# thiviyanT/torch-rgcn

Hardware: AMD Instinct MI355X
Metric: edges/s/GPU (fwd+bwd) 2-layer RGCN, 1M nodes/10M edges/50 rels, h=16 (higher is better)
Workload: dtype f32; 1 GPU; S1: N=1000000 nodes, E=10000000 base triples, R0=50 relations (layer R=101), M=21000000 messages/layer, hidden=16, 2 NC layers (horizontal, vertical), fwd+bwd, learnable X

## Files before the change

include/rgcn_hip.h:

```cpp
#ifndef RGCN_HIP_H
#define RGCN_HIP_H

#include <stdint.h>

#ifdef __cplusplus
extern "C" {
#endif

#define RGCN_API __attribute__((visibility("default")))

#define RGCN_OK 0
#define RGCN_EINVAL 1
#define RGCN_ENOMEM 2
#define RGCN_ERANGE 3
#define RGCN_EHIP 4
#define RGCN_EUNSUPPORTED 5

#define RGCN_CHUNK 16

RGCN_API const char *rgcn_version(void);
RGCN_API const char *rgcn_last_error(void);
RGCN_API const char *rgcn_csrc_sha(void);
RGCN_API int rgcn_poison_lds(void *stream);
RGCN_API int rgcn_set_option(const char *name, int32_t value);
// ... 77 lines not shown
                           int32_t d_out, int32_t flags, void *stream);

RGCN_API int rgcn_pack_w16_f32(const float *W, float *Wp, int32_t R, void *stream);
RGCN_API int rgcn_pack_w_blocks_f32(const float *W, float *Wp, int32_t R, int32_t d_in, int32_t d_out, void *stream);

RGCN_API int rgcn_spmm_scatter_f32(const float *X, const float *Wp, float *Y, const int32_t *p_src,
                                   const float *p_val, const int32_t *p_pos, const int32_t *chunk_rel,
                                   const int32_t *items, int64_t n_items, int32_t d, void *stream);
RGCN_API int rgcn_segment_sum_f32(const float *Y, const int32_t *rowptr, const float *bias, float *out,
                                  int64_t n_rows, int32_t d, int32_t flags, void *stream);
RGCN_API int rgcn_segment_gather_sum_f32(const float *Y, const int32_t *perm, const int32_t *rowptr, const float *bias,
                                         float *out, int64_t n_rows, int32_t d, int32_t flags, void *stream);
RGCN_API int rgcn_segment_gather_sum_units_f32(const float *Y, const int32_t *perm, const int32_t *units, int64_t n_units,
                                               int64_t n_split, const float *bias, float *out, int64_t n_rows, int32_t d,
                                               int32_t flags, void *stream);

RGCN_API int rgcn_wgrad_f32(const float *X, const float *G, float *dW, const int32_t *p_src,
                            const int32_t *p_dst, const float *p_val, const int32_t *chunk_rel,
                            const int32_t *items, int64_t n_items, int64_t n_dst, int64_t n_src, int32_t R,
                            int32_t d_in, int32_t d_out, void *stream);

RGCN_API int rgcn_wgrad_tiled_f32(const float *X, const float *G, float *dW, const int32_t *p_src,
                                  const int32_t *p_dst, const float *p_val, const int32_t *chunk_rel,
                                  const int32_t *run_ptr, int64_t n_tiles, int32_t tile_rows, int64_t n_dst,
                                  int64_t n_src, int32_t R, int32_t d_in, int32_t d_out,
                                  int32_t tiles_per_item, void *stream);

#define RGCN_F_DW_ATOMIC 4
#define RGCN_F_TRANSPOSE_W 8
#define RGCN_F_DIAG4 16
#define RGCN_F_PARTIAL 32
#define RGCN_F_ACCUMULATE 64
RGCN_API int64_t rgcn_bwd_fused_scratch_floats(int64_t n_tiles, int32_t R);
RGCN_API int64_t rgcn_bwd_lean_slot_bytes(int64_t n_chunks);
RGCN_API int rgcn_bwd_lean_prepare_f32(const int32_t *p_pack, const int32_t *chunk_rel, int64_t n_chunks, void *slots, int32_t *hdr,
                                       void *stream);
RGCN_API int rgcn_bwd_lean_prepare_unpacked_f32(const int32_t *p_src, const int32_t *p_dst, const float *p_val, int32_t tile_rows,
                                                const int32_t *chunk_rel, int64_t n_chunks, void *slots, int32_t *hdr, void *stream);
RGCN_API int rgcn_bwd_lean_supported(int32_t tile_rows);
RGCN_API int rgcn_bwd_lean_f32(const float *G, const float *X, const float *Wt_packed, float *dX, float *dW, float *scratch,
                               const void *slots, const int32_t *hdr, const int32_t *run_ptr, int64_t n_tiles, int32_t tile_rows,
                               int64_t n_dst, int32_t R, int32_t flags, void *stream);
RGCN_API int32_t rgcn_bwd_blk_max_rows(int32_t R, int32_t flags);
RGCN_API int rgcn_bwd_blk_supported(int32_t tile_rows, int32_t R, int32_t flags);
RGCN_API int64_t rgcn_bwd_blk_rec_bytes(int64_t n_chunks);
RGCN_API int rgcn_bwd_blk_prepare_f32(const int32_t *p_pack, const int32_t *p_src, const int32_t *p_dst, const float *p_val,
                                      int32_t tile_rows, const int32_t *chunk_rel, int64_t n_chunks, void *rec, void *stream);
RGCN_API int rgcn_bwd_blk_f32(const float *G, const float *X, const float *Wt_packed, float *dX, float *dW, const void *rec,
                              const int32_t *run_ptr, int64_t n_tiles, int32_t tile_rows, int64_t n_dst, int32_t R, int32_t flags,
                              float *dbias, int64_t n_src, const int32_t *units, int64_t n_units, int64_t n_split, void *stream);
RGCN_API int32_t rgcn_bwd_own_waves(void);
RGCN_API int32_t rgcn_bwd_own_units(void);
RGCN_API int32_t rgcn_bwd_own_max_rows(void);
RGCN_API int rgcn_bwd_own_f32(const float *G, const float *X, const float *Wt_packed, float *dX, float *dW, const void *rec,
                              const int32_t *own_ptr, const int32_t *unit_rel, int64_t n_tiles, int32_t tile_rows, int64_t n_dst,
                              int32_t R, int32_t flags, float *dbias, int64_t n_src, void *stream);
RGCN_API int rgcn_bwd_own_bf16(const uint16_t *G, const uint16_t *X, const float *Wt_packed, uint16_t *dX, float *dW, const void *rec,
                               const int32_t *own_ptr, const int32_t *unit_rel, int64_t n_tiles, int32_t tile_rows, int64_t n_dst,
                               int32_t R, int32_t flags, float *dbias, int64_t n_src, void *stream);
RGCN_API int64_t rgcn_softwin_tmp_bytes(int64_t n);
RGCN_API int rgcn_softwin_order(const int32_t *dst, const int32_t *src, const int32_t *rel, const uint8_t *alive, int64_t M, int64_t n_dst,
                                int64_t n_src, int32_t R, int32_t tile_rows, uint64_t *keys, uint64_t *keys_sorted, int32_t *order,
                                int32_t *order_sorted, int32_t *bucket_cnt, int32_t *bucket_base, int32_t *bucket_first, void *tmp,
                                int64_t tmp_bytes, void *stream);
RGCN_API int rgcn_softwin_fill(const int32_t *dst, const int32_t *src, const float *val, const uint64_t *keys_sorted, const int32_t *order_sorted,
                               int64_t n_live, int64_t n_dst, int64_t n_src, int32_t R, int32_t tile_rows, const int32_t *bucket_base,
                               const int32_t *bucket_first, int64_t m_pad, const int32_t *parts, const int32_t *unit_base,
                               const int32_t *unit_owner, const int32_t *unit_local, int32_t own_waves, int32_t *s_src, int32_t *s_dst, float *s_val,
                               uint64_t *ckeys, uint64_t *ckeys_sorted, int32_t *cidx, int32_t *cidx_sorted, int32_t *crel, int32_t *group_cnt,
                               int32_t *p_src, int32_t *p_dst, float *p_val, int32_t *chunk_rel, int32_t *group_ptr, void *tmp, int64_t tmp_bytes,
                               void *stream);
RGCN_API int32_t rgcn_spmm_blk_max_rows(void);
RGCN_API int rgcn_spmm_blk_f32(const float *X, const float *W_packed, const float *bias, float *out, const void *rec,
                               const int32_t *run_ptr, int64_t n_tiles, int32_t tile_rows, int64_t n_dst, int32_t R, int32_t flags,
                               const int32_t *units, int64_t n_units, int64_t n_split, void *stream);
RGCN_API int rgcn_spmm_blk_bf16(const uint16_t *X, const float *W_packed, const float *bias, uint16_t *out, float *scratch, const void *rec,
                                const int32_t *run_ptr, int64_t n_tiles, int32_t tile_rows, int64_t n_dst, int64_t n_src, int32_t R,
                                int32_t flags, const int32_t *units, int64_t n_units, int64_t n_split, void *stream);
RGCN_API int rgcn_spmm_bf16(const uint16_t *X, const float *W_packed, const float *bias, uint16_t *out, float *scratch,
                            const int32_t *p_pack, const int32_t *chunk_rel, const int32_t *units, int64_t n_units, int64_t n_split,
                            int32_t tile_rows, int64_t n_dst, int64_t n_src, int32_t d_in, int32_t d_out, int32_t flags, void *stream);
RGCN_API int rgcn_wgrad_bf16(const uint16_t *X, const uint16_t *G, float *dW, const int32_t *p_src, const int32_t *p_dst,
                             const float *p_val, const int32_t *chunk_rel, const int32_t *items, int64_t n_items, int32_t R,
                             int32_t d_in, int32_t d_out, void *stream);
RGCN_API int rgcn_colsum_bf16(const uint16_t *G, float *db, float *scratch, int64_t n, int32_t d, void *stream);
RGCN_API int rgcn_block_spmm_bf16(const uint16_t *X, const float *blocks, const float *bias, uint16_t *out, float *scratch,
                                  const int32_t *units, const int32_t *rowptr, int64_t n_units, int64_t n_split, const int32_t *e_src,
                                  const int32_t *e_rel, const float *e_val, int64_t n_rows, int32_t n_rel_blocks, int32_t nb, int32_t bi,
                                  int32_t bo, int32_t flags, void *stream);
RGCN_API int rgcn_block_wgrad_bf16(const uint16_t *X, const uint16_t *G, float *dblocks, const int32_t *p_src, const int32_t *p_dst,
                                   const float *p_val, const int32_t *chunk_rel, const int32_t *items, int64_t n_items,
                                   int32_t n_rel_blocks, int32_t nb, int32_t bi, int32_t bo, void *stream);
RGCN_API int rgcn_diag_spmm_bf16(const uint16_t *X, const float *w, const float *bias, uint16_t *out, float *scratch,
                                 const int32_t *rowptr_units, int64_t n_units, int64_t n_split, const int32_t *e_src, const int32_t *e_rel,
                                 const float *e_val, int64_t n_rows, int32_t R, int32_t d, void *stream);
RGCN_API int rgcn_diag_wgrad_bf16(const uint16_t *X, const uint16_t *G, float *dw, const int32_t *p_src, const int32_t *p_dst,
                                  const float *p_val, const int32_t *chunk_rel, const int32_t *items, int64_t n_items, int32_t R, int32_t d,
                                  void *stream);
RGCN_API int rgcn_bwd_scatter_dw_f32(const float *G, const float *X, const float *Wt_packed, float *Y, float *dW,
                                     const int32_t *p_src, const int32_t *p_dst, const float *p_val,
                                     const int32_t *chunk_rel, const int32_t *items, int64_t n_items, int32_t R, int32_t d,
                                     int32_t flags, void *stream);
RGCN_API int rgcn_pack_w16t_f32(const float *W, float *Wp, int32_t R, void *stream);
RGCN_API int rgcn_pack_w16_pair_f32(const float *W, float *Wp, float *Wtp, int32_t R, void *stream);

RGCN_API int rgcn_featureless_fwd_f32(const float *table, const float *bias, float *out, const int32_t *p_src,
                                      const int32_t *p_dst, const float *p_val, const int32_t *chunk_rel,
                                      const int32_t *units, int64_t n_units, int64_t n_split, int32_t tile_rows,
                                      int64_t n_dst, int64_t n_src, int32_t R, int32_t d_out, void *stream);

RGCN_API int rgcn_spmm_csr_d16_supported(int32_t R);
RGCN_API int rgcn_spmm_csr_d16_f32(const float *X, const float *W, const float *bias, float *out, const int32_t *units, int64_t n_units,
// ... 152 lines not shown
```

torch-rgcn_amd/csrc/rgcn_bwd_own.hip:

```cpp
#include <stdlib.h>
#include <string.h>

#include <algorithm>

#include "rgcn_device.h"

namespace {

constexpr int OWN_REC = 176;
constexpr int OWN_REC_ROWS = 128;
constexpr int OWN_REC_HDR = 160;
constexpr int OWN_LDS_MAX = 160 * 1024;
#ifndef RGCN_OWN_NW
#define RGCN_OWN_NW 16
#define RGCN_OWN_K 8
#define RGCN_OWN_U 2
#endif
constexpr int OWN_NW = RGCN_OWN_NW;
constexpr int OWN_K = RGCN_OWN_K;
constexpr int OWN_U = RGCN_OWN_U;
constexpr int OWN_MAX_ROWS = (OWN_LDS_MAX - OWN_NW * BW_SCR2 * 4 - 64) / 192;

typedef float own_acc32 __attribute__((ext_vector_type(32)));

size_t bwd_own_lds(int rows) { return (size_t)rows * 192 + (size_t)OWN_NW * BW_SCR2 * 4 + 64; }

template <bool RELU, int NW, int K, int ABL = 0, bool BF = false>
__global__ __launch_bounds__(64 * NW) void bwd_own_d16_kernel(
    const float *__restrict__ G, const float *__restrict__ X, const float *__restrict__ Wtp, float *__restrict__ dX,
    float *__restrict__ dWout, const char *__restrict__ rec, const int *__restrict__ own_ptr, int n_tiles, int tile_rows, int n_dst,
    float *__restrict__ dbias, int n_src, const int *__restrict__ unit_rel) {
  constexpr int U = OWN_U, NT = 64 * NW;
  constexpr int TQ = (OWN_MAX_ROWS * 4 + NT - 1) / NT;
  static_assert(K <= 9, "8 indexed accumulators + 1");
  constexpr bool EXT = K == 9;
  extern __shared__ __attribute__((aligned(16))) char lds[];
  const int tid = threadIdx.x;
  const int wave = __builtin_amdgcn_readfirstlane(tid >> 6), lane = tid & 63;
  const unsigned xt_off = (unsigned)tile_rows * 128u;
  const unsigned xs_off = (unsigned)tile_rows * 192u;
  float4 *dxz = reinterpret_cast<float4 *>(lds);
  const double2 *dxd2 = reinterpret_cast<const double2 *>(lds);
  float4 *xt4 = reinterpret_cast<float4 *>(lds + xt_off);
  float *xs = reinterpret_cast<float *>(lds + xs_off) + wave * BW_SCR2;

  int t = blockIdx.x;
  int row0 = t * tile_rows;
  int nrows = min(tile_rows, n_dst - row0);
  int c0 = own_ptr[(size_t)t * NW + wave], c1 = own_ptr[(size_t)t * NW + wave + 1];
  c0 = __builtin_amdgcn_readfirstlane(c0);
  c1 = __builtin_amdgcn_readfirstlane(c1);
  float4 gs = make_float4(0.f, 0.f, 0.f, 0.f);
  const long long g_n4 = dbias ? (long long)n_src * 4 : 0, g_step = (long long)gridDim.x * NT;
  long long g_i = (long long)blockIdx.x * NT + tid;
#pragma unroll
  for (int q = 0; q < TQ; ++q) {
    const int idx = tid + q * NT;
    if (idx < tile_rows * 4) {
      float4 x0 = make_float4(0.f, 0.f, 0.f, 0.f);
      if (idx < nrows * 4) {
        if constexpr (BF) x0 = bf16x4_widen(reinterpret_cast<const uint2 *>(X)[(size_t)row0 * 4 + idx]);
        else x0 = reinterpret_cast<const float4 *>(X + (size_t)row0 * 16)[idx];
      }
      xt4[idx] = x0;
    }
  }
  for (int i = tid; i < tile_rows * 8; i += NT) dxz[i] = make_float4(0.f, 0.f, 0.f, 0.f);
  __syncthreads();

  const int m = lane & 15, k = lane >> 4;
  const unsigned kofs = (unsigned)k << 4;
  const unsigned dx_lane = (unsigned)m * 8u;
  const unsigned xrd = xt_off + (unsigned)m * 4u;
  float *xs_wr = xs + m * 16 + 4 * ((k + (m >> 2)) & 3);
  const float *xs_rd = xs + (4 * k) * 16 + 4 * (((m >> 2) + k) & 3) + (m & 3);
  const unsigned slot_lane = (unsigned)m * 8u;
  const unsigned rows_lane = (unsigned)OWN_REC_ROWS + (unsigned)k * 8u;
  const unsigned w_lane = (unsigned)lane * 16u;

  own_acc32 accs;
#pragma unroll
  for (int i = 0; i < 32; ++i) accs[i] = 0.f;
  f32x4 acc8 = f32x4{0.f, 0.f, 0.f, 0.f};

  uint2 sl_n[U], rw_n[U];
  int hd_n[U];
  auto request_idx = [&](int c, int last) {
#pragma unroll
    for (int j = 0; j < U; ++j) {
      const int cc = min(c + j, last);
      const char *r = rec + (size_t)cc * OWN_REC;
      sl_n[j] = *reinterpret_cast<const uint2 *>(r + slot_lane);
      rw_n[j] = *reinterpret_cast<const uint2 *>(r + rows_lane);
      hd_n[j] = *reinterpret_cast<const int *>(r + OWN_REC_HDR);
    }
  };
  if (c0 < c1) request_idx(c0, c1 - 1);

  for (;;) {
    const int last = c1 - 1;
    for (int c = c0; c < c1; c += U) {
      unsigned w0_[U];
      uint2 rw_[U];
      float v_[U];
      int hd_[U];
      float4 g_[U], w_[U];
#pragma unroll
// ... 60 lines not shown
#pragma unroll
          for (int t4 = 0; t4 < 4; ++t4) bv[jj][t4] = xs_rd[16 * t4];
#pragma unroll
          for (int t4 = 0; t4 < 4; ++t4) av[jj][t4] = *reinterpret_cast<const float *>(lds + (xrd + ro[j][t4]));
          asm volatile("" ::: "memory");
        }
#pragma unroll
        for (int jj = 0; jj < P; ++jj) {
          if (h + jj >= U) break;
          const int lr = (ABL & 4) ? 0 : (int)((unsigned)hd_[h + jj] >> 16);
          const bool ext = EXT && lr >= 8;
          const int li = 4 * (lr & 7);
          const f32x4 in0 = f32x4{accs[li], accs[li + 1], accs[li + 2], accs[li + 3]};
          f32x4 aw = EXT ? f32x4{ext ? acc8[0] : in0[0], ext ? acc8[1] : in0[1], ext ? acc8[2] : in0[2], ext ? acc8[3] : in0[3]} : in0;
#pragma unroll
          for (int t4 = 0; t4 < 4; ++t4) aw = __builtin_amdgcn_mfma_f32_16x16x4f32(av[jj][t4], bv[jj][t4], aw, 0, 0, 0);
          accs[li] = ext ? in0[0] : aw[0];
          accs[li + 1] = ext ? in0[1] : aw[1];
          accs[li + 2] = ext ? in0[2] : aw[2];
          accs[li + 3] = ext ? in0[3] : aw[3];
          if (EXT) acc8 = f32x4{ext ? aw[0] : acc8[0], ext ? aw[1] : acc8[1], ext ? aw[2] : acc8[2], ext ? aw[3] : acc8[3]};
        }
      }
#pragma unroll
      for (int j = 0; j < U && !(ABL & 8); ++j)
#pragma unroll
        for (int e = 0; e < 4; ++e)
          __hip_atomic_fetch_add(static_cast<double *>(__builtin_assume_aligned(lds + (dx_lane + 2u * ro[j][e]), 8)), (double)acc[j][e], __ATOMIC_RELAXED,
                                 __HIP_MEMORY_SCOPE_WORKGROUP);
      __builtin_amdgcn_sched_barrier(0);
    }
    const int tn = t + (int)gridDim.x;
    int c0n = 0, c1n = 0, row0n = 0, nrn = 0;
    float4 xn[TQ];
#pragma unroll
    for (int q = 0; q < TQ; ++q) xn[q] = make_float4(0.f, 0.f, 0.f, 0.f);
    if (tn < n_tiles) {
      row0n = tn * tile_rows;
      nrn = min(tile_rows, n_dst - row0n);
      c0n = __builtin_amdgcn_readfirstlane(own_ptr[(size_t)tn * NW + wave]);
      c1n = __builtin_amdgcn_readfirstlane(own_ptr[(size_t)tn * NW + wave + 1]);
#pragma unroll
      for (int q = 0; q < TQ; ++q)
        if (tid + q * NT < nrn * 4) {
          if constexpr (BF) {
            const uint2 u = reinterpret_cast<const uint2 *>(X)[(size_t)row0n * 4 + tid + q * NT];
            xn[q] = make_float4(__uint_as_float(u.x), __uint_as_float(u.y), 0.f, 0.f);
          } else {
            xn[q] = reinterpret_cast<const float4 *>(X + (size_t)row0n * 16)[tid + q * NT];
          }
        }
      if (c0n < c1n) request_idx(c0n, c1n - 1);
    }
    float4 gn = make_float4(0.f, 0.f, 0.f, 0.f);
    if (g_i < g_n4) {
      if constexpr (BF) gn = bf16x4_widen(reinterpret_cast<const uint2 *>(G)[g_i]);
      else gn = reinterpret_cast<const float4 *>(G)[g_i];
    }
    g_i += g_step;
    lds_barrier();
    gs.x += gn.x; gs.y += gn.y; gs.z += gn.z; gs.w += gn.w;
#pragma unroll
    for (int q = 0; q < TQ; ++q) asm volatile("" : "+v"(xn[q].x), "+v"(xn[q].y), "+v"(xn[q].z), "+v"(xn[q].w));
#pragma unroll
    for (int q = 0; q < TQ; ++q) {
      const int idx = tid + q * NT;
      if (idx < nrows * 4) {
        const double2 d0 = dxd2[2 * idx], d1 = dxd2[2 * idx + 1];
        float4 a = make_float4((float)d0.x, (float)d0.y, (float)d1.x, (float)d1.y);
        if (RELU) {
          const float4 x = xt4[idx];
          a.x = x.x > 0.f ? a.x : 0.f; a.y = x.y > 0.f ? a.y : 0.f; a.z = x.z > 0.f ? a.z : 0.f; a.w = x.w > 0.f ? a.w : 0.f;
        }
        if constexpr (BF) reinterpret_cast<uint2 *>(dX)[(size_t)row0 * 4 + idx] = bf16x4_round(a);
        else reinterpret_cast<float4 *>(dX + (size_t)row0 * 16)[idx] = a;
      }
    }
    if (tn >= n_tiles) break;
#pragma unroll
    for (int q = 0; q < TQ; ++q) {
      const int idx = tid + q * NT;
      if (idx < tile_rows * 4) {
        dxz[2 * idx] = make_float4(0.f, 0.f, 0.f, 0.f);
        dxz[2 * idx + 1] = make_float4(0.f, 0.f, 0.f, 0.f);
        if constexpr (BF) xt4[idx] = bf16x4_widen(uint2{__float_as_uint(xn[q].x), __float_as_uint(xn[q].y)});
        else xt4[idx] = xn[q];
      }
    }
    lds_barrier();
    t = tn; row0 = row0n; nrows = nrn; c0 = c0n; c1 = c1n;
  }
  if (dbias) {
    for (; g_i < g_n4; g_i += g_step) {
      float4 gn;
      if constexpr (BF) gn = bf16x4_widen(reinterpret_cast<const uint2 *>(G)[g_i]);
      else gn = reinterpret_cast<const float4 *>(G)[g_i];
      gs.x += gn.x; gs.y += gn.y; gs.z += gn.z; gs.w += gn.w;
    }
#pragma unroll
    for (int sft = 4; sft < 64; sft <<= 1) {
      gs.x += __shfl_xor(gs.x, sft); gs.y += __shfl_xor(gs.y, sft); gs.z += __shfl_xor(gs.z, sft); gs.w += __shfl_xor(gs.w, sft);
    }
    __syncthreads();
    if (lane < 4) *reinterpret_cast<float4 *>(xs + 4 * lane) = gs;
    __syncthreads();
    if (tid < 16) {
      float a = 0.f;
      const float *all = reinterpret_cast<const float *>(lds + xs_off);
      for (int i = 0; i < NW; ++i) a += all[i * BW_SCR2 + tid];
      atomicAdd(dbias + tid, a);
    }
  }
#pragma unroll
  for (int li = 0; li < K; ++li) {
    const int r = __builtin_amdgcn_readfirstlane(unit_rel[wave * K + li]);
    if (r >= 0) {
      float *o = dWout + (size_t)r * 256 + (4 * k) * 16 + m;
      atomicAdd(o, li < 8 ? accs[(4 * li) & 31] : acc8[0]);
      atomicAdd(o + 16, li < 8 ? accs[(4 * li + 1) & 31] : acc8[1]);
      atomicAdd(o + 32, li < 8 ? accs[(4 * li + 2) & 31] : acc8[2]);
      atomicAdd(o + 48, li < 8 ? accs[(4 * li + 3) & 31] : acc8[3]);
    }
  }
}

}

extern "C" int32_t rgcn_bwd_own_waves(void) { return OWN_NW; }
extern "C" int32_t rgcn_bwd_own_units(void) { return OWN_NW * OWN_K; }
extern "C" int32_t rgcn_bwd_own_max_rows(void) { return OWN_MAX_ROWS; }

extern "C" int rgcn_bwd_own_f32(const float *G, const float *X, const float *Wt_packed, float *dX, float *dW, const void *rec,
                                const int32_t *own_ptr, const int32_t *unit_rel, int64_t n_tiles, int32_t tile_rows, int64_t n_dst,
                                int32_t R, int32_t flags, float *dbias, int64_t n_src, void *stream) {
  if (!G || !X || !Wt_packed || !dX || !dW || !rec || !own_ptr || !unit_rel || n_tiles <= 0 || tile_rows <= 0 || n_dst <= 0 || R <= 0 ||
      R > 0xFFFF || n_dst > INT32_MAX || n_tiles * (int64_t)OWN_NW >= INT32_MAX) {
    rgcn_set_error("bwd_own: bad argument");
    return RGCN_EINVAL;
  }
  if (tile_rows > rgcn_bwd_own_max_rows()) {
    rgcn_set_error("bwd_own: tiles of at most %d rows (got %d)", rgcn_bwd_own_max_rows(), tile_rows);
    return RGCN_EUNSUPPORTED;
  }
  if (dbias && (n_src <= 0 || n_src >= (int64_t(1) << 29))) { rgcn_set_error("bwd_own: dbias needs 0 < n_src < 2^29"); return RGCN_EINVAL; }
  hipStream_t st = (hipStream_t)stream;
  int dev = 0, n_cu = 0;
  HIP_TRY(launch_device(&dev, &n_cu));
  HIP_TRY(zero_dw_dbias_async(dW, (size_t)R, dbias, st));
  const size_t lds = bwd_own_lds(tile_rows);
  const unsigned n_blocks = (unsigned)std::min<int64_t>(n_tiles, n_cu);
  auto launch = [&](auto k) -> hipError_t {
    constexpr auto kern = decltype(k)::value;
    hipError_t e = allow_lds<kern>(dev, lds, OWN_LDS_MAX);
    if (e != hipSuccess) return e;
    hipLaunchKernelGGL(kern, dim3(n_blocks), dim3(64 * OWN_NW), lds, st, G, X, Wt_packed, dX, dW, static_cast<const char *>(rec), own_ptr, (int)n_tiles,
                       tile_rows, (int)n_dst, dbias, (int)n_src, unit_rel);
    return hipGetLastError();
  };
#ifdef RGCN_ABLATIONS
  {
    const int ABLV = rgcn_option_value(RGCN_OPT_BWD_ABL);
    if (ABLV == 2) HIP_TRY(launch(kern_c<bwd_own_d16_kernel<false, OWN_NW, OWN_K, 2>>));
    else if (ABLV == 4) HIP_TRY(launch(kern_c<bwd_own_d16_kernel<false, OWN_NW, OWN_K, 4>>));
    else if (ABLV == 8) HIP_TRY(launch(kern_c<bwd_own_d16_kernel<false, OWN_NW, OWN_K, 8>>));
    else if (ABLV == 16) HIP_TRY(launch(kern_c<bwd_own_d16_kernel<false, OWN_NW, OWN_K, 16>>));
    else if (ABLV == 6) HIP_TRY(launch(kern_c<bwd_own_d16_kernel<false, OWN_NW, OWN_K, 6>>));
    else HIP_TRY(launch(kern_c<bwd_own_d16_kernel<false, OWN_NW, OWN_K, 0>>));
    return RGCN_OK;
  }
#endif
  if (flags & RGCN_F_RELU) HIP_TRY(launch(kern_c<bwd_own_d16_kernel<true, OWN_NW, OWN_K>>));
  else HIP_TRY(launch(kern_c<bwd_own_d16_kernel<false, OWN_NW, OWN_K>>));
  return RGCN_OK;
}

extern "C" int rgcn_bwd_own_bf16(const uint16_t *G, const uint16_t *X, const float *Wt_packed, uint16_t *dX, float *dW, const void *rec,
                                 const int32_t *own_ptr, const int32_t *unit_rel, int64_t n_tiles, int32_t tile_rows, int64_t n_dst,
                                 int32_t R, int32_t flags, float *dbias, int64_t n_src, void *stream) {
  if (!G || !X || !Wt_packed || !dX || !dW || !rec || !own_ptr || !unit_rel || n_tiles <= 0 || tile_rows <= 0 || n_dst <= 0 || R <= 0 ||
      R > 0xFFFF || n_dst > INT32_MAX || n_tiles * (int64_t)OWN_NW >= INT32_MAX || n_src <= 0 || n_src >= (int64_t(1) << 26) || flags != 0) {
    rgcn_set_error("bwd_own_bf16: bad argument (the records address G rows as src << 6 in 32 bits: n_src < 2^26; no flags)");
    return RGCN_EINVAL;
  }
  if (tile_rows > rgcn_bwd_own_max_rows()) {
    rgcn_set_error("bwd_own_bf16: tiles of at most %d rows (got %d)", rgcn_bwd_own_max_rows(), tile_rows);
    return RGCN_EUNSUPPORTED;
  }
  hipStream_t st = (hipStream_t)stream;
  int dev = 0, n_cu = 0;
  HIP_TRY(launch_device(&dev, &n_cu));
  HIP_TRY(zero_dw_dbias_async(dW, (size_t)R, dbias, st));
  const size_t lds = bwd_own_lds(tile_rows);
  const unsigned n_blocks = (unsigned)std::min<int64_t>(n_tiles, n_cu);
  auto launch = [&](auto k) -> hipError_t {
    constexpr auto kern = decltype(k)::value;
    hipError_t e = allow_lds<kern>(dev, lds, OWN_LDS_MAX);
    if (e != hipSuccess) return e;
    hipLaunchKernelGGL(kern, dim3(n_blocks), dim3(64 * OWN_NW), lds, st, reinterpret_cast<const float *>(G), reinterpret_cast<const float *>(X),
                       Wt_packed, reinterpret_cast<float *>(dX), dW, static_cast<const char *>(rec), own_ptr, (int)n_tiles, tile_rows, (int)n_dst,
                       dbias, (int)n_src, unit_rel);
    return hipGetLastError();
  };
  HIP_TRY(launch(kern_c<bwd_own_d16_kernel<false, OWN_NW, OWN_K, 0, true>>));
  return RGCN_OK;
}
```

torch-rgcn_amd/torch_rgcn/_native.py:

```python
import ctypes
import re
import threading
import os

import numpy as np
import torch

from . import routes

_LIB_PATH = os.environ.get("RGCN_HIP_LIB") or os.path.join(os.path.dirname(os.path.abspath(__file__)), "lib", "librgcn_hip.so")
_HEADER_PATH = os.path.join(os.path.dirname(os.path.abspath(__file__)), "..", "..", "include", "rgcn_hip.h")
_lib = None

OK, EINVAL, ENOMEM, ERANGE, EHIP, EUNSUPPORTED = range(6)
CHUNK = 16

c_i64 = ctypes.c_int64
_CTYPES = {"int": ctypes.c_int, "int32_t": ctypes.c_int32, "int64_t": ctypes.c_int64, "uint64_t": ctypes.c_uint64}


class NativeLibraryError(RuntimeError):
    pass


# ... 1332 lines not shown
            if cached[2] == 0:
                cached = (None, plan.n_tiles, 0)
        plan._blk_units = cached
    return cached


def _lean_plan(plan):
    lean = getattr(plan, "_lean", None)
    if lean is None:
        n_chunks = plan.chunk_rel.shape[0]
        dev = plan.chunk_rel.device
        slots = torch.empty(int(lib().rgcn_bwd_lean_slot_bytes(n_chunks)) + 16, device=dev, dtype=torch.uint8)
        hdr = torch.empty(max(n_chunks, 1), device=dev, dtype=torch.int32)
        with _on(dev):
            if plan.pack is not None:
                _check(lib().rgcn_bwd_lean_prepare_f32(_dp(plan.pack), _dp(plan.chunk_rel), n_chunks, _dp(slots), _dp(hdr), _stream(dev)),
                       "bwd_lean_prepare")
            else:
                _check(lib().rgcn_bwd_lean_prepare_unpacked_f32(_dp(plan.src), _dp(plan.dst), _dp(plan.val), plan.tile_rows,
                                                                _dp(plan.chunk_rel), n_chunks, _dp(slots), _dp(hdr), _stream(dev)),
                       "bwd_lean_prepare_unpacked")
        lean = plan._lean = (slots, hdr)
    return lean


def _blk_rec(plan):
    rec = getattr(plan, "_blk_rec", None)
    if rec is None:
        n_chunks = plan.chunk_rel.shape[0]
        dev = plan.chunk_rel.device
        rec = torch.empty(int(lib().rgcn_bwd_blk_rec_bytes(n_chunks)) + 16, device=dev, dtype=torch.uint8)
        packed = plan.pack is not None and plan.tile_rows <= 255
        with _on(dev):
            _check(lib().rgcn_bwd_blk_prepare_f32(_dp(plan.pack) if packed else None, _dp(plan.src), _dp(plan.dst), _dp(plan.val),
                                                  plan.tile_rows, _dp(plan.chunk_rel), n_chunks, _dp(rec), _stream(dev)),
                   "bwd_blk_prepare")
        plan._blk_rec = rec
    return rec


def bwd_own_geometry():
    L = lib()
    nw = int(L.rgcn_bwd_own_waves())
    return nw, int(L.rgcn_bwd_own_units()) // nw, int(L.rgcn_bwd_own_max_rows())


def bwd_own_rows(n_nodes, device=None):
    if n_nodes < _BLK_MIN_NODES:
        return 0
    cap = min(bwd_own_geometry()[2], int(routes.get("own_rows_cap", "767")))
    return _even_tile_rows(n_nodes, cap, device)


def bwd_own(G, X, W, plan, relu=False, want_db=False):
    _req(G, "grad_output"); _req(X, "features"); _req(W, "weights")
    assert W.shape[1:] == (16, 16) and G.shape == (plan.n_src, 16) and X.shape == (plan.n_dst, 16) and W.shape[0] == plan.num_rels
    assert getattr(plan, "own_ptr", None) is not None, "bwd_own: a plan made with build_softwin_plan(own_waves=...)"
    dev = G.device
    Wtp = pack_w16t(W)
    dX = torch.empty((plan.n_dst, 16), device=dev, dtype=torch.float32)
    buf = torch.empty(W.numel() + 16, device=dev, dtype=torch.float32)
    dW, db = buf[:W.numel()].view_as(W), buf[W.numel():]
    rec = _blk_rec(plan)
    with _on(dev), _timed("bwd_fused"):
        _check(lib().rgcn_bwd_own_f32(_dp(G), _dp(X), _dp(Wtp), _dp(dX), _dp(dW), _dp(rec), _dp(plan.own_ptr), _dp(plan.unit_rel),
                                      plan.n_tiles, plan.tile_rows, plan.n_dst, W.shape[0], F_RELU if relu else 0,
                                      _dp(db) if want_db else None, plan.n_src, _stream(dev)), "bwd_own")
    return (dX, dW, db if want_db else None)


def bwd_own_bf16(G, X, W, plan, relu=False, want_db=False):
    _req(G, "grad_output", torch.bfloat16); _req(X, "features", torch.bfloat16); _req(W, "weights")
    assert W.shape[1:] == (16, 16) and G.shape == (plan.n_src, 16) and X.shape == (plan.n_dst, 16) and W.shape[0] == plan.num_rels
    assert getattr(plan, "own_ptr", None) is not None, "bwd_own_bf16: a plan made with build_softwin_plan(own_waves=...)"
    dev = G.device
    Wtp = pack_w16t(W)
    dX = torch.empty((plan.n_dst, 16), device=dev, dtype=torch.bfloat16)
    buf = torch.empty(W.numel() + 16, device=dev, dtype=torch.float32)
    dW, db = buf[:W.numel()].view_as(W), buf[W.numel():]
    rec = _blk_rec(plan)
    with _on(dev), _timed("bwd_own_bf16"):
        _check(lib().rgcn_bwd_own_bf16(_dp(G), _dp(X), _dp(Wtp), _dp(dX), _dp(dW), _dp(rec), _dp(plan.own_ptr), _dp(plan.unit_rel), plan.n_tiles,
                                       plan.tile_rows, plan.n_dst, W.shape[0], F_RELU if relu else 0, _dp(db) if want_db else None, plan.n_src,
                                       _stream(dev)), "bwd_own_bf16")
    return (dX, dW, db if want_db else None)


def bwd_fused_relu_ok(plan, diag4=False):
    return bool(_bwd_blk_plan(plan, diag4)) or bwd_fused_ok(plan, diag4)


def bwd_fused(G, X, W, plan, atomic=False, relu=False, want_db=False, diag4=False):
    _req(G, "grad_output"); _req(X, "features"); _req(W, "weights")
    assert W.shape[1:] == (16, 16) and G.shape == (plan.n_src, 16) and X.shape == (plan.n_dst, 16)
    dev = G.device
    Wtp = pack_w16t(W)
    dX = torch.empty((plan.n_dst, 16), device=dev, dtype=torch.float32)
    blk = _bwd_blk_plan(plan, diag4)
    if diag4 and not blk:
        raise NativeLibraryError("bwd_fused: diag4 needs the block-tile kernel (plan of tall tiles, non-deterministic mode)")
    db = None
    if blk and want_db:
        buf = torch.empty(W.numel() + 16, device=dev, dtype=torch.float32)
        dW, db = buf[:W.numel()].view_as(W), buf[W.numel():]
    else:
        dW = torch.empty_like(W)
    ret = (lambda: (dX, dW, db)) if want_db else (lambda: (dX, dW))
    scratch = None
    if not atomic:
        n = int(lib().rgcn_bwd_fused_scratch_floats(plan.n_tiles, W.shape[0]))
        scratch = torch.empty(n, device=dev, dtype=torch.float32)
    if blk:
        if not atomic:
            raise NativeLibraryError("bwd_fused: the block-tile plan (tall tiles) has no bit-reproducible kernel")
        rec = _blk_rec(plan)
        units, n_units, n_split = _blk_units(plan)
        with _on(dev), _timed("bwd_fused"):
            _check(lib().rgcn_bwd_blk_f32(_dp(G), _dp(X), _dp(Wtp), _dp(dX), _dp(dW), _dp(rec), _dp(plan.run_ptr), plan.n_tiles,
                                          plan.tile_rows, plan.n_dst, W.shape[0],
                                          (F_RELU if relu else 0) | (F_DIAG4 if diag4 else 0), _dp(db), plan.n_src, _dp(units),
                                          n_units, n_split, _stream(dev)), "bwd_blk")
        return ret()
    if not (lib().rgcn_bwd_lean_supported(plan.tile_rows) and W.shape[0] < 65536):
        raise NativeLibraryError(f"bwd_fused: no fused kernel for wave-owned tiles of {plan.tile_rows} rows (bwd_fused_ok)")
    slots, hdr = _lean_plan(plan)
    with _on(dev), _timed("bwd_fused"):
        _check(lib().rgcn_bwd_lean_f32(_dp(G), _dp(X), _dp(Wtp), _dp(dX), _dp(dW), _dp(scratch), _dp(slots), _dp(hdr),
                                       _dp(plan.run_ptr), plan.n_tiles, plan.tile_rows, plan.n_dst, W.shape[0],
                                       (F_DW_ATOMIC if atomic else 0) | (1 if relu else 0), _stream(dev)), "bwd_lean")
    return ret()


def bwd_fused_slabs_ok(plan):
    return bool(_bwd_blk_plan(plan)) and _blk_units(plan)[2] == 0 and getattr(plan, "tile_ptr", None) is not None


def bwd_fused_slabs(G, X, W, plan, n_slabs, after_slab):
# ... 495 lines not shown
```

Before: 6.636 billion edges/s.

## Replace dW/dbias atomics in owner backward with per-block partials plus reduce kernel

The owner-partitioned backward kernel now writes each block's per-unit dW accumulators and dbias partial sums to a scratch buffer instead of issuing global atomicAdds, and a new reduction kernel sums them per relation. This also drops the memset that zeroed dW/dbias up front. The dbias G streaming is split across up to TQ loads per tile iteration so the bias sum covers G in fewer passes. The cost is an extra kernel launch, a scratch allocation per call, and a reduce that scans all units for every relation.

```diff
diff --git a/include/rgcn_hip.h b/include/rgcn_hip.h
--- a/include/rgcn_hip.h
+++ b/include/rgcn_hip.h
@@ -153,12 +153,21 @@
 RGCN_API int32_t rgcn_bwd_own_waves(void);
 RGCN_API int32_t rgcn_bwd_own_units(void);
 RGCN_API int32_t rgcn_bwd_own_max_rows(void);
+RGCN_API int64_t rgcn_bwd_own_scratch_floats(int64_t n_tiles);
 RGCN_API int rgcn_bwd_own_f32(const float *G, const float *X, const float *Wt_packed, float *dX, float *dW, const void *rec,
                               const int32_t *own_ptr, const int32_t *unit_rel, int64_t n_tiles, int32_t tile_rows, int64_t n_dst,
                               int32_t R, int32_t flags, float *dbias, int64_t n_src, void *stream);
+RGCN_API int rgcn_bwd_own_part_f32(const float *G, const float *X, const float *Wt_packed, float *dX, float *dW, const void *rec,
+                                   const int32_t *own_ptr, const int32_t *unit_rel, int64_t n_tiles, int32_t tile_rows, int64_t n_dst,
+                                   int32_t R, int32_t flags, float *dbias, int64_t n_src, float *scratch, int64_t scratch_floats,
+                                   void *stream);
 RGCN_API int rgcn_bwd_own_bf16(const uint16_t *G, const uint16_t *X, const float *Wt_packed, uint16_t *dX, float *dW, const void *rec,
                                const int32_t *own_ptr, const int32_t *unit_rel, int64_t n_tiles, int32_t tile_rows, int64_t n_dst,
                                int32_t R, int32_t flags, float *dbias, int64_t n_src, void *stream);
+RGCN_API int rgcn_bwd_own_part_bf16(const uint16_t *G, const uint16_t *X, const float *Wt_packed, uint16_t *dX, float *dW, const void *rec,
+                                    const int32_t *own_ptr, const int32_t *unit_rel, int64_t n_tiles, int32_t tile_rows, int64_t n_dst,
+                                    int32_t R, int32_t flags, float *dbias, int64_t n_src, float *scratch, int64_t scratch_floats,
+                                    void *stream);
 RGCN_API int64_t rgcn_softwin_tmp_bytes(int64_t n);
 RGCN_API int rgcn_softwin_order(const int32_t *dst, const int32_t *src, const int32_t *rel, const uint8_t *alive, int64_t M, int64_t n_dst,
                                 int64_t n_src, int32_t R, int32_t tile_rows, uint64_t *keys, uint64_t *keys_sorted, int32_t *order,
diff --git a/torch-rgcn_amd/csrc/rgcn_bwd_own.hip b/torch-rgcn_amd/csrc/rgcn_bwd_own.hip
--- a/torch-rgcn_amd/csrc/rgcn_bwd_own.hip
+++ b/torch-rgcn_amd/csrc/rgcn_bwd_own.hip
@@ -2,6 +2,7 @@
 #include <string.h>
 
 #include <algorithm>
+#include <type_traits>
 
 #include "rgcn_device.h"
 
@@ -20,17 +21,24 @@
 constexpr int OWN_K = RGCN_OWN_K;
 constexpr int OWN_U = RGCN_OWN_U;
 constexpr int OWN_MAX_ROWS = (OWN_LDS_MAX - OWN_NW * BW_SCR2 * 4 - 64) / 192;
+constexpr int OWN_TQ = (OWN_MAX_ROWS * 4 + 64 * OWN_NW - 1) / (64 * OWN_NW);
+constexpr int OWN_UNITS = OWN_NW * OWN_K;
+constexpr int OWN_PART_BLOCK = OWN_UNITS * 256;
+#ifndef RGCN_OWN_AB
+#define RGCN_OWN_AB 0
+#endif
 
 typedef float own_acc32 __attribute__((ext_vector_type(32)));
 
 size_t bwd_own_lds(int rows) { return (size_t)rows * 192 + (size_t)OWN_NW * BW_SCR2 * 4 + 64; }
 
-template <bool RELU, int NW, int K, int ABL = 0, bool BF = false>
+template <bool RELU, int NW, int K, int ABL = 0, bool BF = false, bool PART = false>
 __global__ __launch_bounds__(64 * NW) void bwd_own_d16_kernel(
     const float *__restrict__ G, const float *__restrict__ X, const float *__restrict__ Wtp, float *__restrict__ dX,
     float *__restrict__ dWout, const char *__restrict__ rec, const int *__restrict__ own_ptr, int n_tiles, int tile_rows, int n_dst,
-    float *__restrict__ dbias, int n_src, const int *__restrict__ unit_rel) {
+    float *__restrict__ dbias, int n_src, const int *__restrict__ unit_rel, float *__restrict__ part, int g_share) {
   constexpr int U = OWN_U, NT = 64 * NW;
+  typedef std::conditional_t<BF, uint2, float4> g_raw;
   constexpr int TQ = (OWN_MAX_ROWS * 4 + NT - 1) / NT;
   static_assert(K <= 9, "8 indexed accumulators + 1");
   constexpr bool EXT = K == 9;
@@ -53,6 +61,13 @@
   float4 gs = make_float4(0.f, 0.f, 0.f, 0.f);
   const long long g_n4 = dbias ? (long long)n_src * 4 : 0, g_step = (long long)gridDim.x * NT;
   long long g_i = (long long)blockIdx.x * NT + tid;
+  const g_raw *Gq = reinterpret_cast<const g_raw *>(G);
+  auto gs_add = [&](const g_raw &v) {
+    float4 f;
+    if constexpr (BF) f = bf16x4_widen(v);
+    else f = v;
+    gs.x += f.x; gs.y += f.y; gs.z += f.z; gs.w += f.w;
+  };
 #pragma unroll
   for (int q = 0; q < TQ; ++q) {
     const int idx = tid + q * NT;
@@ -219,14 +234,18 @@
         }
       if (c0n < c1n) request_idx(c0n, c1n - 1);
     }
-    float4 gn = make_float4(0.f, 0.f, 0.f, 0.f);
-    if (g_i < g_n4) {
-      if constexpr (BF) gn = bf16x4_widen(reinterpret_cast<const uint2 *>(G)[g_i]);
-      else gn = reinterpret_cast<const float4 *>(G)[g_i];
-    }
-    g_i += g_step;
+    g_raw gn[TQ];
+#pragma unroll
+    for (int q = 0; q < TQ; ++q) {
+      gn[q] = g_raw{};
+      if (q < g_share) {
+        if (g_i < g_n4) gn[q] = Gq[g_i];
+        g_i += g_step;
+      }
+    }
     lds_barrier();
-    gs.x += gn.x; gs.y += gn.y; gs.z += gn.z; gs.w += gn.w;
+#pragma unroll
+    for (int q = 0; q < TQ; ++q) gs_add(gn[q]);
 #pragma unroll
     for (int q = 0; q < TQ; ++q) asm volatile("" : "+v"(xn[q].x), "+v"(xn[q].y), "+v"(xn[q].z), "+v"(xn[q].w));
 #pragma unroll
@@ -258,12 +277,7 @@
     t = tn; row0 = row0n; nrows = nrn; c0 = c0n; c1 = c1n;
   }
   if (dbias) {
-    for (; g_i < g_n4; g_i += g_step) {
-      float4 gn;
-      if constexpr (BF) gn = bf16x4_widen(reinterpret_cast<const uint2 *>(G)[g_i]);
-      else gn = reinterpret_cast<const float4 *>(G)[g_i];
-      gs.x += gn.x; gs.y += gn.y; gs.z += gn.z; gs.w += gn.w;
-    }
+    for (; g_i < g_n4; g_i += g_step) gs_add(Gq[g_i]);
 #pragma unroll
     for (int sft = 4; sft < 64; sft <<= 1) {
       gs.x += __shfl_xor(gs.x, sft); gs.y += __shfl_xor(gs.y, sft); gs.z += __shfl_xor(gs.z, sft); gs.w += __shfl_xor(gs.w, sft);
@@ -275,13 +289,19 @@
       float a = 0.f;
       const float *all = reinterpret_cast<const float *>(lds + xs_off);
       for (int i = 0; i < NW; ++i) a += all[i * BW_SCR2 + tid];
-      atomicAdd(dbias + tid, a);
+      if constexpr (PART) part[(size_t)gridDim.x * (NW * K * 256) + (size_t)blockIdx.x * 16 + tid] = a;
+      else atomicAdd(dbias + tid, a);
     }
   }
 #pragma unroll
   for (int li = 0; li < K; ++li) {
     const int r = __builtin_amdgcn_readfirstlane(unit_rel[wave * K + li]);
-    if (r >= 0) {
+    if constexpr (PART) {
+      if (r >= 0) {
+        float *o = part + ((size_t)blockIdx.x * (NW * K) + wave * K + li) * 256 + lane * 4;
+        *reinterpret_cast<f32x4 *>(o) = li < 8 ? f32x4{accs[(4 * li) & 31], accs[(4 * li + 1) & 31], accs[(4 * li + 2) & 31], accs[(4 * li + 3) & 31]} : acc8;
+      }
+    } else if (r >= 0) {
       float *o = dWout + (size_t)r * 256 + (4 * k) * 16 + m;
       atomicAdd(o, li < 8 ? accs[(4 * li) & 31] : acc8[0]);
       atomicAdd(o + 16, li < 8 ? accs[(4 * li + 1) & 31] : acc8[1]);
@@ -291,83 +311,160 @@
   }
 }
 
-}
-
-extern "C" int32_t rgcn_bwd_own_waves(void) { return OWN_NW; }
-extern "C" int32_t rgcn_bwd_own_units(void) { return OWN_NW * OWN_K; }
-extern "C" int32_t rgcn_bwd_own_max_rows(void) { return OWN_MAX_ROWS; }
-
-extern "C" int rgcn_bwd_own_f32(const float *G, const float *X, const float *Wt_packed, float *dX, float *dW, const void *rec,
-                                const int32_t *own_ptr, const int32_t *unit_rel, int64_t n_tiles, int32_t tile_rows, int64_t n_dst,
-                                int32_t R, int32_t flags, float *dbias, int64_t n_src, void *stream) {
+__global__ __launch_bounds__(256) void own_reduce_kernel(const float *__restrict__ part, const int *__restrict__ unit_rel, float *__restrict__ dW,
+                                                         float *__restrict__ dbias, int n_blocks, int n_units, int R) {
+  __shared__ float4 red[16 * 16];
+  float *redf = reinterpret_cast<float *>(red);
+  const int r = blockIdx.x, q = blockIdx.y, tid = threadIdx.x;
+  const int col = tid & 15, s = tid >> 4;
+  if (r == R) {
+    if (q) return;
+    const float *gsp = part + (size_t)n_blocks * n_units * 256;
+    float a = 0.f;
+    for (int b = s; b < n_blocks; b += 16) a += gsp[(size_t)b * 16 + col];
+    redf[s * 16 + col] = a;
+    __syncthreads();
+    if (tid < 16) {
+      float t = 0.f;
+      for (int i = 0; i < 16; ++i) t += redf[i * 16 + tid];
+      dbias[tid] = t;
+    }
+    return;
+  }
+  const float4 *p = reinterpret_cast<const float4 *>(part) + 16 * q + col;
+  const size_t bstep = (size_t)n_units * 64;
+  float4 a = make_float4(0.f, 0.f, 0.f, 0.f);
+  for (int u = 0; u < n_units; ++u) {
+    if (unit_rel[u] != r) continue;
+    const float4 *pu = p + (size_t)u * 64;
+    int b = s;
+    for (; b + 48 < n_blocks; b += 64) {
+      const float4 v0 = pu[(size_t)b * bstep], v1 = pu[(size_t)(b + 16) * bstep], v2 = pu[(size_t)(b + 32) * bstep], v3 = pu[(size_t)(b + 48) * bstep];
+      a.x += v0.x; a.y += v0.y; a.z += v0.z; a.w += v0.w;
+      a.x += v1.x; a.y += v1.y; a.z += v1.z; a.w += v1.w;
+      a.x += v2.x; a.y += v2.y; a.z += v2.z; a.w += v2.w;
+      a.x += v3.x; a.y += v3.y; a.z += v3.z; a.w += v3.w;
+    }
+    for (; b < n_blocks; b += 16) {
+      const float4 v = pu[(size_t)b * bstep];
+      a.x += v.x; a.y += v.y; a.z += v.z; a.w += v.w;
+    }
+  }
+  red[s * 16 + col] = a;
+  __syncthreads();
+  if (tid < 64) {
+    const int e = tid >> 4;
+    float t = 0.f;
+    for (int i = 0; i < 16; ++i) t += redf[(i * 16 + col) * 4 + e];
+    dW[(size_t)r * 256 + (4 * q + e) * 16 + col] = t;
+  }
+}
+
+int64_t own_scratch_floats(int64_t n_tiles, int n_cu) { return std::min<int64_t>(n_tiles, n_cu) * (OWN_PART_BLOCK + 16); }
+
+template <bool BF>
+int bwd_own_run(const char *who, const void *G, const void *X, const float *Wt_packed, void *dX, float *dW, const void *rec, const int32_t *own_ptr,
+                const int32_t *unit_rel, int64_t n_tiles, int32_t tile_rows, int64_t n_dst, int32_t R, int32_t flags, float *dbias, int64_t n_src,
+                float *scratch, int64_t scratch_floats, void *stream) {
   if (!G || !X || !Wt_packed || !dX || !dW || !rec || !own_ptr || !unit_rel || n_tiles <= 0 || tile_rows <= 0 || n_dst <= 0 || R <= 0 ||
-      R > 0xFFFF || n_dst > INT32_MAX || n_tiles * (int64_t)OWN_NW >= INT32_MAX) {
-    rgcn_set_error("bwd_own: bad argument");
+      R > 0xFFFF || n_dst > INT32_MAX || n_tiles * (int64_t)OWN_NW >= INT32_MAX || ((BF || dbias) && n_src <= 0) || n_src >= (int64_t(1) << 26) ||
+      (BF && flags != 0)) {
+    rgcn_set_error("%s: bad argument (the records address G rows as src << 6 in 32 bits: n_src < 2^26%s)", who, BF ? "; no flags" : "");
     return RGCN_EINVAL;
   }
   if (tile_rows > rgcn_bwd_own_max_rows()) {
-    rgcn_set_error("bwd_own: tiles of at most %d rows (got %d)", rgcn_bwd_own_max_rows(), tile_rows);
+    rgcn_set_error("%s: tiles of at most %d rows (got %d)", who, rgcn_bwd_own_max_rows(), tile_rows);
     return RGCN_EUNSUPPORTED;
   }
-  if (dbias && (n_src <= 0 || n_src >= (int64_t(1) << 29))) { rgcn_set_error("bwd_own: dbias needs 0 < n_src < 2^29"); return RGCN_EINVAL; }
   hipStream_t st = (hipStream_t)stream;
   int dev = 0, n_cu = 0;
   HIP_TRY(launch_device(&dev, &n_cu));
-  HIP_TRY(zero_dw_dbias_async(dW, (size_t)R, dbias, st));
+  if (scratch && scratch_floats < own_scratch_floats(n_tiles, n_cu)) {
+    rgcn_set_error("%s: scratch of %lld floats, rgcn_bwd_own_scratch_floats(%lld) = %lld", who, (long long)scratch_floats, (long long)n_tiles,
+                   (long long)own_scratch_floats(n_tiles, n_cu));
+    return RGCN_EINVAL;
+  }
+  if (RGCN_OWN_AB & 1) scratch = nullptr;
+#ifdef RGCN_ABLATIONS
+  const int ABLV = BF ? 0 : rgcn_option_value(RGCN_OPT_BWD_ABL);
+  if (ABLV) scratch = nullptr;
+#endif
+  if (!scratch) HIP_TRY(zero_dw_dbias_async(dW, (size_t)R, dbias, st));
   const size_t lds = bwd_own_lds(tile_rows);
   const unsigned n_blocks = (unsigned)std::min<int64_t>(n_tiles, n_cu);
+  const int64_t g_cover = ((n_tiles + n_blocks - 1) / n_blocks) * (int64_t)n_blocks * 64 * OWN_NW;
+  const int g_share = (RGCN_OWN_AB & 2) || !dbias ? 1 : (int)std::min<int64_t>(OWN_TQ, std::max<int64_t>(1, (n_src * 4 + g_cover - 1) / g_cover));
   auto launch = [&](auto k) -> hipError_t {
     constexpr auto kern = decltype(k)::value;
     hipError_t e = allow_lds<kern>(dev, lds, OWN_LDS_MAX);
     if (e != hipSuccess) return e;
-    hipLaunchKernelGGL(kern, dim3(n_blocks), dim3(64 * OWN_NW), lds, st, G, X, Wt_packed, dX, dW, static_cast<const char *>(rec), own_ptr, (int)n_tiles,
-                       tile_rows, (int)n_dst, dbias, (int)n_src, unit_rel);
+    hipLaunchKernelGGL(kern, dim3(n_blocks), dim3(64 * OWN_NW), lds, st, static_cast<const float *>(G), static_cast<const float *>(X), Wt_packed,
+                       static_cast<float *>(dX), dW, static_cast<const char *>(rec), own_ptr, (int)n_tiles, tile_rows, (int)n_dst, dbias, (int)n_src,
+                       unit_rel, scratch, g_share);
     return hipGetLastError();
   };
+  if constexpr (BF) {
+    if (scratch) HIP_TRY(launch(kern_c<bwd_own_d16_kernel<false, OWN_NW, OWN_K, 0, true, true>>));
+    else HIP_TRY(launch(kern_c<bwd_own_d16_kernel<false, OWN_NW, OWN_K, 0, true>>));
+  } else {
 #ifdef RGCN_ABLATIONS
-  {
-    const int ABLV = rgcn_option_value(RGCN_OPT_BWD_ABL);
-    if (ABLV == 2) HIP_TRY(launch(kern_c<bwd_own_d16_kernel<false, OWN_NW, OWN_K, 2>>));
-    else if (ABLV == 4) HIP_TRY(launch(kern_c<bwd_own_d16_kernel<false, OWN_NW, OWN_K, 4>>));
-    else if (ABLV == 8) HIP_TRY(launch(kern_c<bwd_own_d16_kernel<false, OWN_NW, OWN_K, 8>>));
-    else if (ABLV == 16) HIP_TRY(launch(kern_c<bwd_own_d16_kernel<false, OWN_NW, OWN_K, 16>>));
-    else if (ABLV == 6) HIP_TRY(launch(kern_c<bwd_own_d16_kernel<false, OWN_NW, OWN_K, 6>>));
-    else HIP_TRY(launch(kern_c<bwd_own_d16_kernel<false, OWN_NW, OWN_K, 0>>));
-    return RGCN_OK;
-  }
+    if (ABLV) {
+      if (ABLV == 2) HIP_TRY(launch(kern_c<bwd_own_d16_kernel<false, OWN_NW, OWN_K, 2>>));
+      else if (ABLV == 4) HIP_TRY(launch(kern_c<bwd_own_d16_kernel<false, OWN_NW, OWN_K, 4>>));
+      else if (ABLV == 8) HIP_TRY(launch(kern_c<bwd_own_d16_kernel<false, OWN_NW, OWN_K, 8>>));
+      else if (ABLV == 16) HIP_TRY(launch(kern_c<bwd_own_d16_kernel<false, OWN_NW, OWN_K, 16>>));
+      else if (ABLV == 6) HIP_TRY(launch(kern_c<bwd_own_d16_kernel<false, OWN_NW, OWN_K, 6>>));
+      else HIP_TRY(launch(kern_c<bwd_own_d16_kernel<false, OWN_NW, OWN_K, 0>>));
+      return RGCN_OK;
+    }
 #endif
-  if (flags & RGCN_F_RELU) HIP_TRY(launch(kern_c<bwd_own_d16_kernel<true, OWN_NW, OWN_K>>));
-  else HIP_TRY(launch(kern_c<bwd_own_d16_kernel<false, OWN_NW, OWN_K>>));
+    const bool relu = flags & RGCN_F_RELU;
+    if (scratch) HIP_TRY(relu ? launch(kern_c<bwd_own_d16_kernel<true, OWN_NW, OWN_K, 0, false, true>>) : launch(kern_c<bwd_own_d16_kernel<false, OWN_NW, OWN_K, 0, false, true>>));
+    else HIP_TRY(relu ? launch(kern_c<bwd_own_d16_kernel<true, OWN_NW, OWN_K>>) : launch(kern_c<bwd_own_d16_kernel<false, OWN_NW, OWN_K>>));
+  }
+  if (scratch) {
+    hipLaunchKernelGGL(own_reduce_kernel, dim3((unsigned)R + (dbias ? 1u : 0u), 4), dim3(256), 0, st, scratch, unit_rel, dW, dbias, (int)n_blocks,
+                       OWN_UNITS, R);
+    HIP_TRY(hipGetLastError());
+  }
   return RGCN_OK;
+}
+
+}
+
+extern "C" int32_t rgcn_bwd_own_waves(void) { return OWN_NW; }
+extern "C" int32_t rgcn_bwd_own_units(void) { return OWN_UNITS; }
+extern "C" int32_t rgcn_bwd_own_max_rows(void) { return OWN_MAX_ROWS; }
+
+extern "C" int64_t rgcn_bwd_own_scratch_floats(int64_t n_tiles) {
+  int dev = 0, n_cu = 0;
+  if (n_tiles <= 0) { rgcn_set_error("bwd_own_scratch_floats: bad argument"); return -1; }
+  if (hipError_t e = launch_device(&dev, &n_cu); e != hipSuccess) { rgcn_set_error("bwd_own_scratch_floats: %s", hipGetErrorString(e)); return -1; }
+  return own_scratch_floats(n_tiles, n_cu);
+}
+
+extern "C" int rgcn_bwd_own_f32(const float *G, const float *X, const float *Wt_packed, float *dX, float *dW, const void *rec,
+                                const int32_t *own_ptr, const int32_t *unit_rel, int64_t n_tiles, int32_t tile_rows, int64_t n_dst,
+                                int32_t R, int32_t flags, float *dbias, int64_t n_src, void *stream) {
+  return bwd_own_run<false>("bwd_own", G, X, Wt_packed, dX, dW, rec, own_ptr, unit_rel, n_tiles, tile_rows, n_dst, R, flags, dbias, n_src, nullptr, 0, stream);
+}
+
+extern "C" int rgcn_bwd_own_part_f32(const float *G, const float *X, const float *Wt_packed, float *dX, float *dW, const void *rec,
+                                     const int32_t *own_ptr, const int32_t *unit_rel, int64_t n_tiles, int32_t tile_rows, int64_t n_dst,
+                                     int32_t R, int32_t flags, float *dbias, int64_t n_src, float *scratch, int64_t scratch_floats, void *stream) {
+  return bwd_own_run<false>("bwd_own_part", G, X, Wt_packed, dX, dW, rec, own_ptr, unit_rel, n_tiles, tile_rows, n_dst, R, flags, dbias, n_src, scratch,
+                            scratch_floats, stream);
 }
 
 extern "C" int rgcn_bwd_own_bf16(const uint16_t *G, const uint16_t *X, const float *Wt_packed, uint16_t *dX, float *dW, const void *rec,
                                  const int32_t *own_ptr, const int32_t *unit_rel, int64_t n_tiles, int32_t tile_rows, int64_t n_dst,
                                  int32_t R, int32_t flags, float *dbias, int64_t n_src, void *stream) {
-  if (!G || !X || !Wt_packed || !dX || !dW || !rec || !own_ptr || !unit_rel || n_tiles <= 0 || tile_rows <= 0 || n_dst <= 0 || R <= 0 ||
-      R > 0xFFFF || n_dst > INT32_MAX || n_tiles * (int64_t)OWN_NW >= INT32_MAX || n_src <= 0 || n_src >= (int64_t(1) << 26) || flags != 0) {
-    rgcn_set_error("bwd_own_bf16: bad argument (the records address G rows as src << 6 in 32 bits: n_src < 2^26; no flags)");
-    return RGCN_EINVAL;
-  }
-  if (tile_rows > rgcn_bwd_own_max_rows()) {
-    rgcn_set_error("bwd_own_bf16: tiles of at most %d rows (got %d)", rgcn_bwd_own_max_rows(), tile_rows);
-    return RGCN_EUNSUPPORTED;
-  }
-  hipStream_t st = (hipStream_t)stream;
-  int dev = 0, n_cu = 0;
-  HIP_TRY(launch_device(&dev, &n_cu));
-  HIP_TRY(zero_dw_dbias_async(dW, (size_t)R, dbias, st));
-  const size_t lds = bwd_own_lds(tile_rows);
-  const unsigned n_blocks = (unsigned)std::min<int64_t>(n_tiles, n_cu);
-  auto launch = [&](auto k) -> hipError_t {
-    constexpr auto kern = decltype(k)::value;
-    hipError_t e = allow_lds<kern>(dev, lds, OWN_LDS_MAX);
-    if (e != hipSuccess) return e;
-    hipLaunchKernelGGL(kern, dim3(n_blocks), dim3(64 * OWN_NW), lds, st, reinterpret_cast<const float *>(G), reinterpret_cast<const float *>(X),
-                       Wt_packed, reinterpret_cast<float *>(dX), dW, static_cast<const char *>(rec), own_ptr, (int)n_tiles, tile_rows, (int)n_dst,
-                       dbias, (int)n_src, unit_rel);
-    return hipGetLastError();
-  };
-  HIP_TRY(launch(kern_c<bwd_own_d16_kernel<false, OWN_NW, OWN_K, 0, true>>));
-  return RGCN_OK;
-}
+  return bwd_own_run<true>("bwd_own_bf16", G, X, Wt_packed, dX, dW, rec, own_ptr, unit_rel, n_tiles, tile_rows, n_dst, R, flags, dbias, n_src, nullptr, 0, stream);
+}
+
+extern "C" int rgcn_bwd_own_part_bf16(const uint16_t *G, const uint16_t *X, const float *Wt_packed, uint16_t *dX, float *dW, const void *rec,
+                                      const int32_t *own_ptr, const int32_t *unit_rel, int64_t n_tiles, int32_t tile_rows, int64_t n_dst,
+                                      int32_t R, int32_t flags, float *dbias, int64_t n_src, float *scratch, int64_t scratch_floats, void *stream) {
+  return bwd_own_run<true>("bwd_own_part_bf16", G, X, Wt_packed, dX, dW, rec, own_ptr, unit_rel, n_tiles, tile_rows, n_dst, R, flags, dbias, n_src,
+                           scratch, scratch_floats, stream);
+}
diff --git a/torch-rgcn_amd/torch_rgcn/_native.py b/torch-rgcn_amd/torch_rgcn/_native.py
--- a/torch-rgcn_amd/torch_rgcn/_native.py
+++ b/torch-rgcn_amd/torch_rgcn/_native.py
@@ -1408,7 +1408,17 @@
     return _even_tile_rows(n_nodes, cap, device)
 
 
-def bwd_own(G, X, W, plan, relu=False, want_db=False):
+def _own_scratch(plan, dev):
+    n = getattr(plan, "_own_scratch_n", None)
+    if n is None:
+        n = int(lib().rgcn_bwd_own_scratch_floats(plan.n_tiles))
+        if n < 0:
+            raise NativeLibraryError("bwd_own: " + lib().rgcn_last_error().decode())
+        plan._own_scratch_n = n
+    return torch.empty(n, device=dev, dtype=torch.float32), n
+
+
+def bwd_own(G, X, W, plan, relu=False, want_db=False, partials=True):
     _req(G, "grad_output"); _req(X, "features"); _req(W, "weights")
     assert W.shape[1:] == (16, 16) and G.shape == (plan.n_src, 16) and X.shape == (plan.n_dst, 16) and W.shape[0] == plan.num_rels
     assert getattr(plan, "own_ptr", None) is not None, "bwd_own: a plan made with build_softwin_plan(own_waves=...)"
@@ -1418,14 +1428,21 @@
     buf = torch.empty(W.numel() + 16, device=dev, dtype=torch.float32)
     dW, db = buf[:W.numel()].view_as(W), buf[W.numel():]
     rec = _blk_rec(plan)
-    with _on(dev), _timed("bwd_fused"):
-        _check(lib().rgcn_bwd_own_f32(_dp(G), _dp(X), _dp(Wtp), _dp(dX), _dp(dW), _dp(rec), _dp(plan.own_ptr), _dp(plan.unit_rel),
-                                      plan.n_tiles, plan.tile_rows, plan.n_dst, W.shape[0], F_RELU if relu else 0,
-                                      _dp(db) if want_db else None, plan.n_src, _stream(dev)), "bwd_own")
+    with _on(dev):
+        scratch, n_scratch = _own_scratch(plan, dev) if partials else (None, 0)
+        with _timed("bwd_fused"):
+            if partials:
+                _check(lib().rgcn_bwd_own_part_f32(_dp(G), _dp(X), _dp(Wtp), _dp(dX), _dp(dW), _dp(rec), _dp(plan.own_ptr), _dp(plan.unit_rel),
+                                                   plan.n_tiles, plan.tile_rows, plan.n_dst, W.shape[0], F_RELU if relu else 0,
+                                                   _dp(db) if want_db else None, plan.n_src, _dp(scratch), n_scratch, _stream(dev)), "bwd_own")
+            else:
+                _check(lib().rgcn_bwd_own_f32(_dp(G), _dp(X), _dp(Wtp), _dp(dX), _dp(dW), _dp(rec), _dp(plan.own_ptr), _dp(plan.unit_rel),
+                                              plan.n_tiles, plan.tile_rows, plan.n_dst, W.shape[0], F_RELU if relu else 0,
+                                              _dp(db) if want_db else None, plan.n_src, _stream(dev)), "bwd_own")
     return (dX, dW, db if want_db else None)
 
 
-def bwd_own_bf16(G, X, W, plan, relu=False, want_db=False):
+def bwd_own_bf16(G, X, W, plan, relu=False, want_db=False, partials=True):
     _req(G, "grad_output", torch.bfloat16); _req(X, "features", torch.bfloat16); _req(W, "weights")
     assert W.shape[1:] == (16, 16) and G.shape == (plan.n_src, 16) and X.shape == (plan.n_dst, 16) and W.shape[0] == plan.num_rels
     assert getattr(plan, "own_ptr", None) is not None, "bwd_own_bf16: a plan made with build_softwin_plan(own_waves=...)"
@@ -1435,10 +1452,18 @@
     buf = torch.empty(W.numel() + 16, device=dev, dtype=torch.float32)
     dW, db = buf[:W.numel()].view_as(W), buf[W.numel():]
     rec = _blk_rec(plan)
-    with _on(dev), _timed("bwd_own_bf16"):
-        _check(lib().rgcn_bwd_own_bf16(_dp(G), _dp(X), _dp(Wtp), _dp(dX), _dp(dW), _dp(rec), _dp(plan.own_ptr), _dp(plan.unit_rel), plan.n_tiles,
-                                       plan.tile_rows, plan.n_dst, W.shape[0], F_RELU if relu else 0, _dp(db) if want_db else None, plan.n_src,
-                                       _stream(dev)), "bwd_own_bf16")
+    with _on(dev):
+        scratch, n_scratch = _own_scratch(plan, dev) if partials else (None, 0)
+        with _timed("bwd_own_bf16"):
+            if partials:
+                _check(lib().rgcn_bwd_own_part_bf16(_dp(G), _dp(X), _dp(Wtp), _dp(dX), _dp(dW), _dp(rec), _dp(plan.own_ptr), _dp(plan.unit_rel),
+                                                    plan.n_tiles, plan.tile_rows, plan.n_dst, W.shape[0], F_RELU if relu else 0,
+                                                    _dp(db) if want_db else None, plan.n_src, _dp(scratch), n_scratch, _stream(dev)),
+                       "bwd_own_bf16")
+            else:
+                _check(lib().rgcn_bwd_own_bf16(_dp(G), _dp(X), _dp(Wtp), _dp(dX), _dp(dW), _dp(rec), _dp(plan.own_ptr), _dp(plan.unit_rel),
+                                               plan.n_tiles, plan.tile_rows, plan.n_dst, W.shape[0], F_RELU if relu else 0,
+                                               _dp(db) if want_db else None, plan.n_src, _stream(dev)), "bwd_own_bf16")
     return (dX, dW, db if want_db else None)
 
 
```

New measurement: 6.634 billion edges/s. About the same (-0.0%).
